# hamidthri/navbot_ppo

Measured on AMD Instinct MI355X. Metric: env_steps_per_sec, higher is better.
Workload: dtype f32; 1 GPU; BASELINE configs[1]: 4096 envs/GPU, stage_1 (32 segments), 10 beams, PPO mlp64x2, rollout=512, 50 full-batch epochs, episode cap 500; n_envs_total=4096, n_envs_per_gpu=4096, rollout_len=512, epochs=50, policy=mlp64x2, parallelism=env-shard dp1, update_arith=bf16x3, rollout=persistent kernel (navsim_rollout_mlp64)

## Files before the change

navbot_ppo_amd/csrc/ppo_mlp64_x3s.h:

```cpp
#pragma once

namespace x3s {

typedef unsigned u32x4 __attribute__((ext_vector_type(4)));
typedef unsigned u32x2 __attribute__((ext_vector_type(2)));
typedef short s16x4 __attribute__((ext_vector_type(4)));
typedef float v4f __attribute__((ext_vector_type(4)));

constexpr int SW = 4;
constexpr int kPieceB = 32 * 128;
constexpr int kImgB = 3 * kPieceB;

struct SmemS {
    uint16_t W2p[3][H][H];
    uint16_t W2Tp[3][H][H];
    uint16_t W1p[3][H][16];
    float b1[H], b2[H], w3[H], w4[H];
    unsigned char img[SW][2][kImgB];
};
static_assert(sizeof(SmemS) <= 160 * 1024, "LDS");
static_assert(offsetof(SmemS, img) % 128 == 0 && kImgB % 128 == 0, "image bases keep the low 7 address bits of a lane offset (the XOR swizzles)");
static_assert(sizeof(SmemS::img) >= 4 * ((Layout<16>::P_ACTOR + 6) & ~3) * sizeof(float), "reduction rows fit the images");
static_assert(sizeof(SmemS::img) / SW >= 96 * 64 * sizeof(float), "lane partials fit a wave's images");

#ifndef X3S_GUARD
#define X3S_GUARD ""
#endif
#define X3S_G "s_nop 0\n\t"
#define X3S_MFMA32_V_AV(acc, A, B) asm volatile(X3S_GUARD "v_mfma_f32_32x32x16_bf16 %0, %1, %2, %0" : "+v"(acc) : "a"(A), "v"(B))
#define X3S_MFMA32_V_AA(acc, A, B) asm volatile(X3S_GUARD "v_mfma_f32_32x32x16_bf16 %0, %1, %2, %0" : "+v"(acc) : "a"(A), "a"(B))
#define X3S_MFMA32G_V_AV(acc, A, B) asm volatile(X3S_G "v_mfma_f32_32x32x16_bf16 %0, %1, %2, %0" : "+v"(acc) : "a"(A), "v"(B))
#define X3S_MFMA32G_V_AA(acc, A, B) asm volatile(X3S_G "v_mfma_f32_32x32x16_bf16 %0, %1, %2, %0" : "+v"(acc) : "a"(A), "a"(B))
#define X3S_MFMA32_VZ_AV(acc, A, B) asm volatile(X3S_G "v_mfma_f32_32x32x16_bf16 %0, %1, %2, 0" : "=&v"(acc) : "a"(A), "v"(B))
#define X3S_MFMA32_VZ_AA(acc, A, B) asm volatile(X3S_G "v_mfma_f32_32x32x16_bf16 %0, %1, %2, 0" : "=&v"(acc) : "a"(A), "a"(B))
#define X3S_MFMA32_A_AV(acc, A, B) asm volatile(X3S_GUARD "v_mfma_f32_32x32x16_bf16 %0, %1, %2, %0" : "+a"(acc) : "a"(A), "v"(B))
#define X3S_MFMA32_AZ_AV(acc, A, B) asm volatile(X3S_G "v_mfma_f32_32x32x16_bf16 %0, %1, %2, 0" : "=&a"(acc) : "a"(A), "v"(B))
#define X3S_MFMA32_A_AA(acc, A, B) asm volatile(X3S_GUARD "v_mfma_f32_32x32x16_bf16 %0, %1, %2, %0" : "+a"(acc) : "a"(A), "a"(B))
#define X3S_MFMA16_A_AA(acc, A, B) asm volatile(X3S_GUARD "v_mfma_f32_16x16x32_bf16 %0, %1, %2, %0" : "+a"(acc) : "a"(A), "a"(B))
#define X3S_MFMA16_V_AA(acc, A, B) asm volatile(X3S_GUARD "v_mfma_f32_16x16x32_bf16 %0, %1, %2, %0" : "+v"(acc) : "a"(A), "a"(B))
#define X3S_MFMA16G_V_AA(acc, A, B) asm volatile(X3S_G "v_mfma_f32_16x16x32_bf16 %0, %1, %2, %0" : "+v"(acc) : "a"(A), "a"(B))
#define X3S_MFMA16_A_VA(acc, A, B) asm volatile(X3S_GUARD "v_mfma_f32_16x16x32_bf16 %0, %1, %2, %0" : "+a"(acc) : "v"(A), "a"(B))
#define X3S_MFMA16_V_VA(acc, A, B) asm volatile(X3S_GUARD "v_mfma_f32_16x16x32_bf16 %0, %1, %2, %0" : "+v"(acc) : "v"(A), "a"(B))
#define X3S_MFMA16G_A_AA(acc, A, B) asm volatile(X3S_G "v_mfma_f32_16x16x32_bf16 %0, %1, %2, %0" : "+a"(acc) : "a"(A), "a"(B))
#define X3S_MFMA16_A_AV(acc, A, B) asm volatile(X3S_GUARD "v_mfma_f32_16x16x32_bf16 %0, %1, %2, %0" : "+a"(acc) : "a"(A), "v"(B))

#define X3S_REP10(F, b) F(b + 0); F(b + 1); F(b + 2); F(b + 3); F(b + 4); F(b + 5); F(b + 6); F(b + 7); F(b + 8); F(b + 9);


__device__ __forceinline__ void split_a(unsigned& p0, float& ra, float& rb, const float a, const float b) {
    asm volatile("v_cvt_pk_bf16_f32 %0, %3, %4\n\t"
                 "v_lshlrev_b32 %1, 16, %0\n\t"
                 "v_and_b32 %2, 0xffff0000, %0\n\t"
                 "v_sub_f32 %1, %3, %1\n\t"
                 "v_sub_f32 %2, %4, %2"
                 : "=&v"(p0), "=&v"(ra), "=&v"(rb) : "v"(a), "v"(b));
}
__device__ __forceinline__ void split_b(unsigned& p1, unsigned& p2, const float ra, const float rb) {
    float t0, t1;
    asm volatile("v_cvt_pk_bf16_f32 %0, %4, %5\n\t"
                 "v_lshlrev_b32 %2, 16, %0\n\t"
                 "v_and_b32 %3, 0xffff0000, %0\n\t"
                 "v_sub_f32 %2, %4, %2\n\t"
                 "v_sub_f32 %3, %5, %3\n\t"
                 "v_cvt_pk_bf16_f32 %1, %2, %3"
                 : "=&v"(p1), "=&v"(p2), "=&v"(t0), "=&v"(t1) : "v"(ra), "v"(rb));
}
__device__ __forceinline__ void relu4(float (&h)[16], const f32x16& c, const int g) {
    float y0, y1, y2, y3;
    asm volatile("v_max_i32 %0, %4, 0\n\tv_max_i32 %1, %5, 0\n\tv_max_i32 %2, %6, 0\n\tv_max_i32 %3, %7, 0"
                 : "=&v"(y0), "=&v"(y1), "=&v"(y2), "=&v"(y3) : "v"(c[4 * g]), "v"(c[4 * g + 1]), "v"(c[4 * g + 2]), "v"(c[4 * g + 3]));
    h[4 * g] = y0; h[4 * g + 1] = y1; h[4 * g + 2] = y2; h[4 * g + 3] = y3;
}
template <bool ACTOR>
__device__ __forceinline__ void dot4(float& z3, float& z4, const float (&h)[16], const int g, const v4f w3, const v4f w4) {
    if constexpr (ACTOR)
        asm volatile("v_fmac_f32 %0, %2, %6\n\tv_fmac_f32 %1, %2, %10\n\t"
                     "v_fmac_f32 %0, %3, %7\n\tv_fmac_f32 %1, %3, %11\n\t"
                     "v_fmac_f32 %0, %4, %8\n\tv_fmac_f32 %1, %4, %12\n\t"
                     "v_fmac_f32 %0, %5, %9\n\tv_fmac_f32 %1, %5, %13"
                     : "+v"(z3), "+v"(z4)
                     : "v"(h[4 * g]), "v"(h[4 * g + 1]), "v"(h[4 * g + 2]), "v"(h[4 * g + 3]), "v"(w3.x), "v"(w3.y), "v"(w3.z), "v"(w3.w),
                       "v"(w4.x), "v"(w4.y), "v"(w4.z), "v"(w4.w));
    else
        asm volatile("v_fmac_f32 %0, %1, %5\n\tv_fmac_f32 %0, %2, %6\n\tv_fmac_f32 %0, %3, %7\n\tv_fmac_f32 %0, %4, %8"
                     : "+v"(z3)
                     : "v"(h[4 * g]), "v"(h[4 * g + 1]), "v"(h[4 * g + 2]), "v"(h[4 * g + 3]), "v"(w3.x), "v"(w3.y), "v"(w3.z), "v"(w3.w));
}
template <bool ACTOR>
__device__ __forceinline__ void dh2_value(float& h, float& pw3, float& pw4, float& pb2, const float g3, const float g4, const float w3,
                                          const float w4) {
    float d;
    if constexpr (ACTOR)
        asm volatile("v_fmac_f32 %1, %0, %5\n\t"
                     "v_fmac_f32 %2, %0, %6\n\t"
                     "v_mul_f32 %4, %6, %8\n\t"
                     "v_fmac_f32 %4, %5, %7\n\t"
                     "v_cmp_lt_f32 vcc, 0, %0\n\t"
                     "v_cndmask_b32 %0, 0, %4, vcc\n\t"
                     "v_add_f32 %3, %3, %0"
                     : "+v"(h), "+v"(pw3), "+v"(pw4), "+v"(pb2), "=&v"(d) : "v"(g3), "v"(g4), "v"(w3), "v"(w4) : "vcc");
    else
        asm volatile("v_fmac_f32 %1, %0, %4\n\t"
                     "v_mul_f32 %3, %4, %5\n\t"
                     "v_cmp_lt_f32 vcc, 0, %0\n\t"
                     "v_cndmask_b32 %0, 0, %3, vcc\n\t"
                     "v_add_f32 %2, %2, %0"
                     : "+v"(h), "+v"(pw3), "+v"(pb2), "=&v"(d) : "v"(g3), "v"(w3) : "vcc");
}

__device__ __forceinline__ void mask4(float& y0, float& y1, float& y2, float& y3, const float x0, const float x1, const float x2,
                                      const float x3, const unsigned w0, const unsigned w1) {
    asm volatile("v_cmp_ne_u16 vcc, 0, %8\n\t"
                 "v_cndmask_b32 %0, 0, %4, vcc\n\t"
                 "v_cmp_lt_u32 vcc, 0xffff, %8\n\t"
                 "v_cndmask_b32 %1, 0, %5, vcc\n\t"
                 "v_cmp_ne_u16 vcc, 0, %9\n\t"
                 "v_cndmask_b32 %2, 0, %6, vcc\n\t"
                 "v_cmp_lt_u32 vcc, 0xffff, %9\n\t"
                 "v_cndmask_b32 %3, 0, %7, vcc"
                 : "=&v"(y0), "=&v"(y1), "=&v"(y2), "=&v"(y3) : "v"(x0), "v"(x1), "v"(x2), "v"(x3), "v"(w0), "v"(w1) : "vcc");
}

struct P3 {
    u32x4 p[3];
};

__device__ __forceinline__ int fswz(const int m) { return (m & 3) | ((((m >> 2) ^ (m >> 3)) & 1) << 2) | ((((m >> 1) ^ (m >> 3)) & 1) << 3); }

typedef __attribute__((address_space(3))) s16x4* lds_s16x4;
__device__ __forceinline__ u32x2 tr_read(const unsigned char* p) {
    const s16x4 v = __builtin_amdgcn_ds_read_tr16_b64_v4i16((lds_s16x4)p);
    u32x2 r;
    __builtin_memcpy(&r, &v, 8);
    return r;
}
__device__ __forceinline__ u32x4 cat(const u32x2 lo, const u32x2 hi) { return u32x4{lo.x, lo.y, hi.x, hi.y}; }

template <bool ACTOR>
__device__ __forceinline__ void pass_body(SmemS& sm, const float* __restrict__ params, const unsigned char* __restrict__ prep,
                                          const float* __restrict__ act, const float* __restrict__ logp_old,
                                          const float* __restrict__ rtg, const float* __restrict__ adv, long long M, float var,
                                          float clip, float inv_n, float* __restrict__ partial, float* __restrict__ stats_partial) {
    using L = Layout<16>;
    constexpr int OFF_W1 = L::OFF_W1, OFF_B1 = L::OFF_B1, OFF_W2 = L::OFF_W2, OFF_B2 = L::OFF_B2, OFF_W3 = L::OFF_W3, OFF_B3 = L::OFF_B3,
                  OFF_W4 = L::OFF_W4, OFF_B4 = L::OFF_B4;
    constexpr int P = ACTOR ? L::P_ACTOR : L::P_CRITIC;
    constexpr int NT = 64 * SW, kTileBytes = XPad<16>::kTileBytes, kRowsBytes = XPad<16>::kRowsBytes;
    const int tid = threadIdx.x, lane = tid & 63, wave = __builtin_amdgcn_readfirstlane(tid >> 6);
    const int l31 = lane & 31, lhi = lane >> 5, l15 = lane & 15, kk = lane >> 4;

#ifdef X3S_EXPERIMENT_COPY_PROLOGUE
    for (int k = tid; k < (int)offsetof(SmemS, img) / 16; k += NT)
        reinterpret_cast<u32x4*>(&sm)[k] = reinterpret_cast<const u32x4*>(prep)[k + (ACTOR ? 0 : (int)offsetof(SmemS, img) / 16)];
#else
    for (int k = tid; k < H * H / 2; k += NT) {
        const int r = (2 * k) / H, c = (2 * k) % H;
        uint32_t p0, p1, p2;
        bf16x3::split_pair(params[OFF_W2 + r * H + c], params[OFF_W2 + r * H + c + 1], p0, p1, p2);
        const uint32_t pc[3] = {p0, p1, p2};
#pragma unroll
        for (int i = 0; i < 3; ++i) {
            *reinterpret_cast<uint32_t*>(&sm.W2p[i][0][0] + wslot(r, kpos(c))) = pc[i];
            (&sm.W2Tp[i][0][0])[wslot(c, kpos(r))] = (uint16_t)(pc[i] & 0xffffu);
            (&sm.W2Tp[i][0][0])[wslot(c + 1, kpos(r))] = (uint16_t)(pc[i] >> 16);
        }
    }
    for (int k = tid; k < H * 16 / 2; k += NT) {
        const int r = (2 * k) / 16, c = (2 * k) % 16;
        uint32_t p0, p1, p2;
        bf16x3::split_pair(params[OFF_W1 + r * 16 + c], params[OFF_W1 + r * 16 + c + 1], p0, p1, p2);
        *reinterpret_cast<uint32_t*>(&sm.W1p[0][r][c]) = p0;
        *reinterpret_cast<uint32_t*>(&sm.W1p[1][r][c]) = p1;
        *reinterpret_cast<uint32_t*>(&sm.W1p[2][r][c]) = p2;
    }
    if (tid < H) {
        sm.b1[tid] = params[OFF_B1 + tid];
        sm.b2[tid] = params[OFF_B2 + tid];
        sm.w3[tid] = params[OFF_W3 + tid];
        sm.w4[tid] = ACTOR ? params[OFF_W4 + tid] : 0.f;
    }
#endif
    const float b3 = params[OFF_B3];
    const float b4 = ACTOR ? params[OFF_B4] : 0.f;
    __syncthreads();

    unsigned char* const smb = reinterpret_cast<unsigned char*>(&sm);
    const int img0 = (int)offsetof(SmemS, img) + wave * 2 * kImgB;
    constexpr int IMG_H = 0, IMG_D = kImgB;
    const int st_base = img0 + l31 * 128 + ((fswz(l31) ^ lhi) << 3);
    auto st_off = [&](const int t, const int j, const int b) { return st_base ^ ((8 * t + 4 * j + 2 * b) << 3); };
    const int g_row = 8 * lhi + (l15 >> 2), g_quad = 4 * ((lane >> 4) & 1) + (lane & 3);
    const int g_base0 = img0 + g_row * 128 + ((g_quad ^ fswz(g_row)) << 3), g_base1 = img0 + (g_row + 4) * 128 + ((g_quad ^ fswz(g_row + 4)) << 3);
    auto g_off = [&](const int t, const int s, const int rd) { return ((rd ? g_base1 : g_base0) ^ (t << 6)) + s * 2048; };
    const int h_row = 8 * kk + (l15 >> 2), h_quad = lane & 3;
    const int h_base0 = img0 + h_row * 128 + ((h_quad ^ fswz(h_row)) << 3), h_base1 = img0 + (h_row + 4) * 128 + ((h_quad ^ fswz(h_row + 4)) << 3);
    auto ldw = [&](const uint16_t* base, const int tt, const int s, const int i) {
        return *reinterpret_cast<const u32x4*>(base + i * H * H + wslot(32 * tt + l31, 16 * s + 8 * lhi));
    };
    const int vec_off = 4 * lhi;
    auto ldv = [&](const float* v, const int t, const int g) { return *reinterpret_cast<const v4f*>(v + 32 * t + 8 * g + vec_off); };

    f32x16 aW2[2][2];
    v4f aW1[4], aB1[4];
#pragma unroll
    for (int a = 0; a < 2; ++a)
#pragma unroll
        for (int b = 0; b < 2; ++b) aW2[a][b] = zero16();
#pragma unroll
    for (int u = 0; u < 4; ++u) aW1[u] = aB1[u] = v4f{0.f, 0.f, 0.f, 0.f};
    float pb2[2][16], pw3[2][16], pw4[2][16];
#pragma unroll
    for (int t = 0; t < 2; ++t)
#pragma unroll
        for (int r = 0; r < 16; ++r) pb2[t][r] = pw3[t][r] = pw4[t][r] = 0.f;
    float adb3 = 0.f, adb4 = 0.f, st0 = 0.f, st1 = 0.f, st2 = 0.f, st3 = 0.f;
    auto keep_w2 = [&]() {
        asm volatile("" : "+a"(aW2[0][0]), "+a"(aW2[0][1]), "+a"(aW2[1][0]), "+a"(aW2[1][1]), "+a"(aW1[0]), "+a"(aW1[1]), "+a"(aW1[2]), "+a"(aW1[3]));
    };
    u32x4 ones = {0x3f803f80u, 0x3f803f80u, 0x3f803f80u, 0x3f803f80u};
    asm volatile("" : "+a"(ones));

    const long long n_tiles = (M + 31) / 32;
    const long long gw = (long long)blockIdx.x * SW + wave, stride = (long long)gridDim.x * SW;
    u32x4 xp[3], xbn[3];
    auto keep_cols = [&]() { asm volatile("" : "+a"(xbn[0]), "+a"(xbn[1]), "+a"(xbn[2])); };
    float pre_a0 = 0.f, pre_a1 = 0.f, pre_lp = 0.f, pre_t = 0.f;
    auto request_rows = [&](long long t) {
        asm volatile("" : "+s"(t));
        const unsigned char* r = prep + (size_t)t * kTileBytes + ((l31 * 3) * 16 + 8 * lhi) * 2;
        asm volatile("global_load_dwordx4 %0, %3, off\n\tglobal_load_dwordx4 %1, %3, off offset:32\n\tglobal_load_dwordx4 %2, %3, off offset:64"
                     : "=a"(xp[0]), "=a"(xp[1]), "=a"(xp[2]) : "v"(r));
    };
    auto request_cols = [&](const long long t) {
        const unsigned char* c = prep + (size_t)t * kTileBytes + kRowsBytes + (l15 * 32 + 8 * kk) * 2;
        asm volatile("global_load_dwordx4 %0, %3, off\n\tglobal_load_dwordx4 %1, %3, off offset:1024\n\tglobal_load_dwordx4 %2, %3, off offset:2048"
                     : "=a"(xbn[0]), "=a"(xbn[1]), "=a"(xbn[2]) : "v"(c));
    };
    auto request_scalars = [&](const long long t) {
        if constexpr (ACTOR) {
            const long long m = t * 32 + l31;
            if (m < M) {
                const float2 a = reinterpret_cast<const float2*>(act)[m];
                pre_a0 = a.x;
                pre_a1 = a.y;
                pre_lp = logp_old[m];
                pre_t = adv[m];
            }
        } else {
            int l = l31;
            long long ts = t;
            asm volatile("" : "+v"(l), "+s"(ts));
            const long long m = ts * 32 + l;
            pre_t = rtg[m < M ? m : M - 1];
        }
    };
    auto landed = [&]() {
        asm volatile("s_waitcnt vmcnt(0)" : "+a"(xp[0]), "+a"(xp[1]), "+a"(xp[2]), "+a"(xbn[0]), "+a"(xbn[1]), "+a"(xbn[2]));
    };
    static_assert(kTileBytes == 6144 && kRowsBytes == 3072, "offsets of the asm loads: pieces 32 bytes apart in a row, 1024 in the columns");

    struct G1Ops {
        P3 da[4];
    };
    auto g1_gather_pair = [&](G1Ops& o, const int q, const int hb0, const int hb1) {
        const int u = q / 3, i = q % 3;
        o.da[u].p[i] = cat(tr_read(smb + (hb0 ^ (u << 5)) + IMG_D + i * kPieceB), tr_read(smb + (hb1 ^ (u << 5)) + IMG_D + i * kPieceB));
    };
    auto g1_step = [&](const int k, const G1Ops& o, const u32x4 (&xb)[3], const bool guard = false) {
        const int t1 = k / 18, q = k % 18, u = 2 * t1 + (q & 1), e = q >> 1;
        constexpr int kind[9] = {0, 1, 0, 0, 1, 0, 0, 1, 0};
        constexpr int ai[9] = {2, 2, 1, 0, 1, 1, 0, 0, 0};
        constexpr int bi[9] = {0, 0, 1, 2, 0, 0, 1, 0, 0};
        if (guard) {
            if (kind[e]) { X3S_MFMA16G_V_AA(aB1[u], o.da[u].p[ai[e]], ones); }
            else { X3S_MFMA16G_A_AA(aW1[u], o.da[u].p[ai[e]], xb[bi[e]]); }
        } else {
            if (ACTOR) {
                if (kind[e]) { X3S_MFMA16_V_AA(aB1[u], o.da[u].p[ai[e]], ones); }
                else { X3S_MFMA16_A_AA(aW1[u], o.da[u].p[ai[e]], xb[bi[e]]); }
            } else {
                if (kind[e]) { X3S_MFMA16_V_VA(aB1[u], o.da[u].p[ai[e]], ones); }
                else { X3S_MFMA16_A_VA(aW1[u], o.da[u].p[ai[e]], xb[bi[e]]); }
            }
        }
    };
    auto store_pieces = [&](const int img, const int t, const int j, const P3& q) {
#pragma unroll
        for (int i = 0; i < 3; ++i) {
            *reinterpret_cast<u32x2*>(smb + st_off(t, j, 0) + img + i * kPieceB) = u32x2{q.p[i].x, q.p[i].y};
            *reinterpret_cast<u32x2*>(smb + st_off(t, j, 1) + img + i * kPieceB) = u32x2{q.p[i].z, q.p[i].w};
        }
    };
    struct SplitState {
        float ra[4], rb[4];
    };
    auto split_block = [&](const float (&c)[16], const int j, const int b, P3& q, SplitState& ss) {
        const int pr = b >> 1;
        if ((b & 1) == 0) {
            unsigned p0;
            split_a(p0, ss.ra[pr], ss.rb[pr], c[8 * j + 2 * pr], c[8 * j + 2 * pr + 1]);
            q.p[0][pr] = p0;
        } else {
            unsigned p1, p2;
            split_b(p1, p2, ss.ra[pr], ss.rb[pr]);
            q.p[1][pr] = p1;
            q.p[2][pr] = p2;
        }
    };

    f32x16 c1[2], c2[2];
    float h1[2][16];
    P3 hb[4];
    u32x4 wn[2][3], wa[2][3];
    SplitState ss1;
    auto g2_step = [&](const int k, const P3 (&dA)[2][2], const P3 (&hB)[2][2], f32x16 (&aW2)[2][2]) {
        const int t2 = k / 24, sk = (k / 12) & 1, e = (k % 12) >> 1, t1 = k & 1;
        constexpr int ai[6] = {2, 1, 0, 1, 0, 0}, bi[6] = {0, 1, 2, 0, 1, 0};
        X3S_MFMA32_A_AA(aW2[t2][t1], dA[t2][sk].p[ai[e]], hB[t1][sk].p[bi[e]]);
    };
    auto b1_to_c1 = [&](const int q) {
        const v4f b = ldv(sm.b1, q >> 2, q & 3);
        c1[q >> 2][4 * (q & 3)] = b.x; c1[q >> 2][4 * (q & 3) + 1] = b.y; c1[q >> 2][4 * (q & 3) + 2] = b.z; c1[q >> 2][4 * (q & 3) + 3] = b.w;
    };
    auto b2_to_c2 = [&](const int q) {
        const v4f b = ldv(sm.b2, q >> 2, q & 3);
        c2[q >> 2][4 * (q & 3)] = b.x; c2[q >> 2][4 * (q & 3) + 1] = b.y; c2[q >> 2][4 * (q & 3) + 2] = b.z; c2[q >> 2][4 * (q & 3) + 3] = b.w;
    };
    auto ld_wa = [&](const int t, const int i) { wa[t][i] = *reinterpret_cast<const u32x4*>(&sm.W1p[i][32 * t + l31][8 * lhi]); };
    auto ld_wn = [&](const int t, const int i) { wn[t][i] = ldw(&sm.W2p[0][0][0], t, 0, i); };
    auto f1_mfma = [&](const int j) {
        const int t = j / 6, e = j % 6;
        constexpr int wi[6] = {2, 1, 0, 1, 0, 0}, xi[6] = {0, 1, 2, 0, 1, 0};
        if (e == 0) { X3S_MFMA32G_V_AA(c1[t], wa[t][wi[e]], xp[xi[e]]); } else { X3S_MFMA32_V_AA(c1[t], wa[t][wi[e]], xp[xi[e]]); }
    };
    auto ahead_work = [&](const int n, const bool alone) {
        if (n == 11 || n == 13) ld_wa(0, (n - 11) / 2);
        if (n == 15 || n == 17) ld_wa(1, (n - 15) / 2);
        if (n == 19) { ld_wa(0, 2); ld_wa(1, 2); }
        if (n >= 22 && n <= 29) b1_to_c1(n - 22);
        if (n == 42) { ld_wn(0, 0); ld_wn(1, 0); ld_wn(0, 1); ld_wn(1, 1); }
        if (n == 43) {
            ld_wn(0, 2); ld_wn(1, 2);
            if (alone) asm volatile("s_nop 7" : "+v"(c1[0]));
            relu4(h1[0], c1[0], 0);
        }
        if (n == 44) relu4(h1[0], c1[0], 1);
        if (n >= 45 && n <= 52) { split_block(h1[0], 0, n - 45, hb[0], ss1); b2_to_c2(n - 45); }
        if (n == 53) relu4(h1[0], c1[0], 2);
        if (n == 54) relu4(h1[0], c1[0], 3);
        if (n >= 55 && n <= 58) relu4(h1[1], c1[1], n - 55);
    };

    for (int k = lane; k < kImgB / 16; k += 64) reinterpret_cast<u32x4*>(smb + img0 + IMG_D)[k] = u32x4{0u, 0u, 0u, 0u};
    bool have_prev = false;
    if (gw < n_tiles) {
        request_rows(gw);
        request_cols(gw);
        request_scalars(gw);
        auto slot = [&](const int n) {
            if (n == 36) landed();
            if (n >= 36 && n < 48) f1_mfma(n - 36);
            ahead_work(n, true);
        };
        X3S_REP10(slot, 10) X3S_REP10(slot, 20) X3S_REP10(slot, 30) X3S_REP10(slot, 40) X3S_REP10(slot, 50)
    }
    for (long long tile = gw; tile < n_tiles; tile += stride) {
        const bool valid = tile * 32 + l31 < M;
        const float cur_a0 = pre_a0, cur_a1 = pre_a1, cur_lp = pre_lp, cur_t = pre_t;
        const long long tile1 = tile + stride < n_tiles ? tile + stride : tile;

        G1Ops g1o;
        float h2[2][16];
        float z3 = 0.f, z4 = 0.f;
        {
            u32x4 wk[4][2];
            SplitState ss;
#pragma unroll
            for (int s = 0; s < 3; ++s) {
                u32x4 w[2][3];
#pragma unroll
                for (int i = 0; i < 3; ++i) { w[0][i] = wn[0][i]; w[1][i] = wn[1][i]; }
                keep_w2();
                keep_cols();
                auto filler = [&](const int slot) {
                    if (slot >= 1 && slot <= 8) split_block(h1[(s + 1) >> 1], (s + 1) & 1, slot - 1, hb[s + 1], ss);
                    if (slot == 0 || slot == 4 || slot == 9) {
                        const int i = slot == 0 ? 0 : slot == 4 ? 1 : 2;
                        wn[0][i] = ldw(&sm.W2p[0][0][0], 0, s + 1, i);
                        wn[1][i] = ldw(&sm.W2p[0][0][0], 1, s + 1, i);
                    }
                    if (slot == 9) store_pieces(IMG_H, s >> 1, s & 1, hb[s]);
                };
                if (s == 0) { X3S_MFMA32G_V_AV(c2[0], w[0][2], hb[s].p[0]); } else { X3S_MFMA32_V_AV(c2[0], w[0][2], hb[s].p[0]); }
                filler(0);
                if (s == 0) { X3S_MFMA32G_V_AV(c2[1], w[1][2], hb[s].p[0]); } else { X3S_MFMA32_V_AV(c2[1], w[1][2], hb[s].p[0]); }
                filler(1);
                X3S_MFMA32_V_AV(c2[0], w[0][1], hb[s].p[1]); filler(2);
                X3S_MFMA32_V_AV(c2[1], w[1][1], hb[s].p[1]); filler(3);
                X3S_MFMA32_V_AV(c2[0], w[0][0], hb[s].p[2]); filler(4);
                X3S_MFMA32_V_AV(c2[1], w[1][0], hb[s].p[2]); filler(5);
                X3S_MFMA32_V_AV(c2[0], w[0][1], hb[s].p[0]); filler(6);
                X3S_MFMA32_V_AV(c2[1], w[1][1], hb[s].p[0]); filler(7);
                X3S_MFMA32_V_AV(c2[0], w[0][0], hb[s].p[1]); filler(8);
                X3S_MFMA32_V_AV(c2[1], w[1][0], hb[s].p[1]); filler(9);
            }
            int hb0 = h_base0, hb1 = h_base1;
            asm volatile("" : "+v"(hb0), "+v"(hb1));
            int gq = 0;
            auto gather = [&]() { g1_gather_pair(g1o, gq, hb0, hb1); ++gq; };
            auto ld_wk = [&](const int s, const int t) { wk[s][t] = ldw(&sm.W2p[0][0][0], t, s, 0); };
            keep_w2();
            keep_cols();
            X3S_MFMA32_V_AV(c2[0], wn[0][2], hb[3].p[0]); ld_wk(0, 0); ld_wk(1, 0);
            X3S_MFMA32_V_AV(c2[0], wn[0][1], hb[3].p[1]); ld_wk(2, 0); ld_wk(3, 0);
            X3S_MFMA32_V_AV(c2[0], wn[0][0], hb[3].p[2]); gather(); gather();
            X3S_MFMA32_V_AV(c2[0], wn[0][1], hb[3].p[0]); gather(); gather();
            X3S_MFMA32_V_AV(c2[0], wn[0][0], hb[3].p[1]); gather(); gather();
            X3S_MFMA32_V_AV(c2[0], wk[0][0], hb[0].p[0]); gather(); gather();
            X3S_MFMA32_V_AV(c2[0], wk[1][0], hb[1].p[0]); gather(); gather();
            X3S_MFMA32_V_AV(c2[0], wk[2][0], hb[2].p[0]); gather();
            X3S_MFMA32_V_AV(c2[0], wk[3][0], hb[3].p[0]); gather();
            v4f hw3[4], hw4[4] = {};
            auto ld_hw = [&](const int g) {
                hw3[g] = ldv(sm.w3, 0, g);
                if (ACTOR) hw4[g] = ldv(sm.w4, 0, g);
            };
            X3S_MFMA32_V_AV(c2[1], wn[1][2], hb[3].p[0]); ld_wk(0, 1); ld_wk(1, 1); ld_hw(0);
            X3S_MFMA32_V_AV(c2[1], wn[1][1], hb[3].p[1]); ld_wk(2, 1); ld_wk(3, 1); ld_hw(1);
            X3S_MFMA32_V_AV(c2[1], wn[1][0], hb[3].p[2]); store_pieces(IMG_H, 1, 1, hb[3]);
            X3S_MFMA32_V_AV(c2[1], wn[1][1], hb[3].p[0]); relu4(h2[0], c2[0], 0); relu4(h2[0], c2[0], 1);
            X3S_MFMA32_V_AV(c2[1], wn[1][0], hb[3].p[1]); relu4(h2[0], c2[0], 2); relu4(h2[0], c2[0], 3);
#pragma unroll
            for (int s = 0; s < 4; ++s) {
                X3S_MFMA32_V_AV(c2[1], wk[s][1], hb[s].p[0]);
                dot4<ACTOR>(z3, z4, h2[0], s, hw3[s], hw4[s]);
                if (s < 2) ld_hw(s + 2);
            }
        }

        int g1k = 0;
        keep_w2();
        {
            v4f hw3[4], hw4[4] = {};
            g1_step(g1k++, g1o, xbn);
            hw3[0] = ldv(sm.w3, 1, 0); hw3[1] = ldv(sm.w3, 1, 1);
            if (ACTOR) { hw4[0] = ldv(sm.w4, 1, 0); hw4[1] = ldv(sm.w4, 1, 1); }
            g1_step(g1k++, g1o, xbn);
            hw3[2] = ldv(sm.w3, 1, 2); hw3[3] = ldv(sm.w3, 1, 3);
            if (ACTOR) { hw4[2] = ldv(sm.w4, 1, 2); hw4[3] = ldv(sm.w4, 1, 3); }
            g1_step(g1k++, g1o, xbn);
            relu4(h2[1], c2[1], 0); relu4(h2[1], c2[1], 1);
            g1_step(g1k++, g1o, xbn);
            relu4(h2[1], c2[1], 2); relu4(h2[1], c2[1], 3);
#pragma unroll
            for (int g = 0; g < 4; ++g) {
                g1_step(g1k++, g1o, xbn);
                dot4<ACTOR>(z3, z4, h2[1], g, hw3[g], hw4[g]);
            }
        }
        float g3 = 0.f, g4 = 0.f;
        {
            z3 += __shfl_xor(z3, 32, 64);
            if (ACTOR) z4 += __shfl_xor(z4, 32, 64);
            const float own = (lhi == 0) ? 1.f : 0.f;
            if (valid) {
                z3 += b3;
                z4 += b4;
#ifdef MLP64_DEBUG_Z
                if (lhi == 0) {
                    float* const dbg = partial + (size_t)200 * P;
                    dbg[tile * 32 + l31] = z3;
                    if (ACTOR) dbg[M + tile * 32 + l31] = z4;
                }
#endif
                if (ACTOR) {
                    const float mu0 = 1.0f / (1.0f + expf(-z3));
                    const float mu1 = tanhf(z4);
                    const float d0 = cur_a0 - mu0, d1 = cur_a1 - mu1;
                    const float lp = -0.5f * ((d0 * d0 + d1 * d1) / var) - 1.8378770664093453f - logf(var);
                    const float lr = lp - cur_lp;
                    const float ratio = expf(lr);
                    const float A = cur_t;
                    const float s1 = ratio * A;
                    const float rc = fminf(fmaxf(ratio, 1.0f - clip), 1.0f + clip);
                    const float s2 = rc * A;
                    st0 += own * -fminf(s1, s2);
                    st2 += own * ((ratio - 1.0f) - lr);
                    st3 += (fabsf(ratio - 1.0f) > clip) ? own : 0.f;
                    const bool inside = (ratio >= 1.0f - clip) && (ratio <= 1.0f + clip);
                    const float dL_dratio = (inside || s1 < s2) ? -A : 0.f;
                    const float dL_dlp = dL_dratio * ratio * inv_n;
                    g3 = dL_dlp * (d0 / var) * (mu0 * (1.0f - mu0));
                    g4 = dL_dlp * (d1 / var) * (1.0f - mu1 * mu1);
                } else {
                    const float e = z3 - cur_t;
                    st1 += own * (e * e);
                    g3 = 2.0f * e * inv_n;
                }
            }
            adb3 += own * g3;
            adb4 += own * g4;
#ifdef MLP64_DEBUG_Z
            if (valid && lhi == 0) {
                float* const dbg = partial + (size_t)200 * P;
                dbg[2 * M + tile * 32 + l31] = g3;
                if (ACTOR) dbg[3 * M + tile * 32 + l31] = g4;
            }
#endif
        }
        {
            v4f wn3 = ldv(sm.w3, 0, 0), wn4 = ACTOR ? ldv(sm.w4, 0, 0) : v4f{0.f, 0.f, 0.f, 0.f};
#pragma unroll
            for (int q = 0; q < 8; ++q) {
                const int t = q >> 2, g = q & 3;
                const v4f w = wn3, v = wn4;
                if (q < 7) {
                    wn3 = ldv(sm.w3, (q + 1) >> 2, (q + 1) & 3);
                    if (ACTOR) wn4 = ldv(sm.w4, (q + 1) >> 2, (q + 1) & 3);
                }
                const float wv3[4] = {w.x, w.y, w.z, w.w}, wv4[4] = {v.x, v.y, v.z, v.w};
#pragma unroll
                for (int j = 0; j < 4; ++j) {
                    const int r = 4 * g + j;
                    dh2_value<ACTOR>(h2[t][r], pw3[t][r], pw4[t][r], pb2[t][r], g3, g4, wv3[j], wv4[j]);
                    if (g1k < 36 && (j & 1)) g1_step(g1k++, g1o, xbn);
                }
                if (g1k < 36 && (g & 1)) g1_step(g1k++, g1o, xbn);
            }
        }

        f32x16 c3[2];
        P3 hB[2][2], dA[2][2];
        u32x2 mw[8];
        float d1[2][16];
        auto d_mask = [&](const int k) {
            const int t = k >> 2, r0 = 8 * ((k >> 1) & 1) + 4 * (k & 1);
            mask4(d1[t][r0], d1[t][r0 + 1], d1[t][r0 + 2], d1[t][r0 + 3], c3[t][r0], c3[t][r0 + 1], c3[t][r0 + 2], c3[t][r0 + 3], mw[k].x, mw[k].y);
        };
        {
            P3 db[4];
            u32x4 wk[4][2], wt[2][3];
            SplitState ss;
#pragma unroll
            for (int i = 0; i < 3; ++i) {
                wt[0][i] = ldw(&sm.W2Tp[0][0][0], 0, 0, i);
                wt[1][i] = ldw(&sm.W2Tp[0][0][0], 1, 0, i);
            }
#pragma unroll
            for (int b = 0; b < 8; ++b) {
                g1_step(g1k++, g1o, xbn);
                split_block(h2[0], 0, b, db[0], ss);
            }
#pragma unroll
            for (int s = 0; s < 4; ++s) {
                u32x4 w[2][3];
#pragma unroll
                for (int i = 0; i < 3; ++i) { w[0][i] = wt[0][i]; w[1][i] = wt[1][i]; }
                keep_w2();
                auto filler = [&](const int slot) {
                    if (s == 0 && slot == 0) request_cols(tile);
                    if (s == 0 && slot == 1) request_rows(tile1);
                    if (s == 3 && slot == 0) request_scalars(tile1);
                    if (s < 3 && slot >= 1 && slot <= 8) split_block(h2[(s + 1) >> 1], (s + 1) & 1, slot - 1, db[s + 1], ss);
                    if (s == 3 && slot < 8) wk[slot >> 1][slot & 1] = ldw(&sm.W2Tp[0][0][0], slot & 1, slot >> 1, 0);
                    if (slot == 2 || slot == 5 || slot == 8) {
                        const int q = 3 * s + (slot - 2) / 3, t = q / 6, sk = (q / 3) & 1, i = q % 3;
                        hB[t][sk].p[i] = cat(tr_read(smb + g_off(t, sk, 0) + IMG_H + i * kPieceB), tr_read(smb + g_off(t, sk, 1) + IMG_H + i * kPieceB));
                    }
                    if (s == 3 && (slot == 3 || slot == 4 || slot == 6 || slot == 7)) {
                        const int k0 = 2 * (slot - 3 - (slot > 4));
#pragma unroll
                        for (int k = k0; k < k0 + 2; ++k)
                            mw[k] = *reinterpret_cast<const u32x2*>(smb + st_off(k >> 2, (k >> 1) & 1, k & 1) + IMG_H);
                    }
                    if (s < 3 && (slot == 0 || slot == 4 || slot == 9)) {
                        const int i = slot == 0 ? 0 : slot == 4 ? 1 : 2;
                        wt[0][i] = ldw(&sm.W2Tp[0][0][0], 0, s + 1, i);
                        wt[1][i] = ldw(&sm.W2Tp[0][0][0], 1, s + 1, i);
                    }
                    if (slot == 9) store_pieces(IMG_D, s >> 1, s & 1, db[s]);
                };
                if (s == 0) { X3S_MFMA32_VZ_AV(c3[0], w[0][2], db[s].p[0]); } else { X3S_MFMA32_V_AV(c3[0], w[0][2], db[s].p[0]); }
                filler(0);
                if (s == 0) { X3S_MFMA32_VZ_AV(c3[1], w[1][2], db[s].p[0]); } else { X3S_MFMA32_V_AV(c3[1], w[1][2], db[s].p[0]); }
                filler(1);
                X3S_MFMA32_V_AV(c3[0], w[0][1], db[s].p[1]); filler(2);
                X3S_MFMA32_V_AV(c3[1], w[1][1], db[s].p[1]); filler(3);
                X3S_MFMA32_V_AV(c3[0], w[0][0], db[s].p[2]); filler(4);
                X3S_MFMA32_V_AV(c3[1], w[1][0], db[s].p[2]); filler(5);
                X3S_MFMA32_V_AV(c3[0], w[0][1], db[s].p[0]); filler(6);
                X3S_MFMA32_V_AV(c3[1], w[1][1], db[s].p[0]); filler(7);
                X3S_MFMA32_V_AV(c3[0], w[0][0], db[s].p[1]); filler(8);
                X3S_MFMA32_V_AV(c3[1], w[1][0], db[s].p[1]); filler(9);
            }
            int dq = 0;
            auto gather_d = [&]() {
                const int t = dq / 6, sk = (dq / 3) & 1, i = dq % 3;
                dA[t][sk].p[i] = cat(tr_read(smb + g_off(t, sk, 0) + IMG_D + i * kPieceB), tr_read(smb + g_off(t, sk, 1) + IMG_D + i * kPieceB));
                ++dq;
            };
#pragma unroll
            for (int s = 0; s < 4; ++s) {
                X3S_MFMA32_V_AV(c3[0], wk[s][0], db[s].p[0]);
                gather_d(); gather_d();
            }
#pragma unroll
            for (int s = 0; s < 4; ++s) {
                X3S_MFMA32_V_AV(c3[1], wk[s][1], db[s].p[0]);
                if (s < 2) { gather_d(); gather_d(); }
                else d_mask(s - 2);
            }
        }

        {
            P3 eb[4];
            SplitState ss;
            auto d_work = [&](const int n) {
                if (n == 0 || n == 1) d_mask(2 + n);
                if (n == 20 || n == 21) d_mask(4 + n - 20);
                if (n == 31 || n == 32) d_mask(6 + n - 31);
                const int s = n < 11 ? 0 : n < 20 ? 1 : n < 31 ? 2 : 3, n0 = s == 0 ? 2 : s == 1 ? 11 : s == 2 ? 22 : 33;
                if (n >= n0 && n < n0 + 8) split_block(d1[s >> 1], s & 1, n - n0, eb[s], ss);
                if (n == n0 + 8) store_pieces(IMG_D, s >> 1, s & 1, eb[s]);
            };
            auto slot = [&](const int n) {
                if (n == 36) landed();
                if (n < 36) g2_step(n, dA, hB, aW2);
                else if (n < 48) f1_mfma(n - 36);
                else g2_step(n - 12, dA, hB, aW2);
                d_work(n);
                ahead_work(n, false);
            };
            X3S_REP10(slot, 0) X3S_REP10(slot, 10) X3S_REP10(slot, 20) X3S_REP10(slot, 30) X3S_REP10(slot, 40) X3S_REP10(slot, 50)
        }
        have_prev = true;
    }
    if (have_prev) {
        G1Ops g1o;
#pragma unroll
        for (int q = 0; q < 12; ++q) g1_gather_pair(g1o, q, h_base0, h_base1);
#pragma unroll
        for (int k = 0; k < 36; ++k) g1_step(k, g1o, xbn, true);
    }

    __syncthreads();
    float rb2[2], rw3[2], rw4[2];
    {
        float* const scr = reinterpret_cast<float*>(&sm.img[wave][0][0]);
#pragma unroll
        for (int t = 0; t < 2; ++t)
#pragma unroll
            for (int r = 0; r < 16; ++r) {
                scr[(0 * 32 + 16 * t + r) * 64 + lane] = pb2[t][r];
                scr[(1 * 32 + 16 * t + r) * 64 + lane] = pw3[t][r];
                scr[(2 * 32 + 16 * t + r) * 64 + lane] = pw4[t][r];
            }
        __builtin_amdgcn_fence(__ATOMIC_RELEASE, "wavefront");
        __builtin_amdgcn_wave_barrier();
        const int row = l31, hi = (row >> 2) & 1, r = (row & 3) + 4 * (row >> 3), t = lhi;
        float s[3] = {0.f, 0.f, 0.f};
#pragma unroll
        for (int v = 0; v < 3; ++v) {
            const float* src = scr + (v * 32 + 16 * t + r) * 64 + 32 * hi;
#pragma unroll
            for (int m = 0; m < 32; m += 4) {
                const v4f q = *reinterpret_cast<const v4f*>(src + m);
                s[v] += (q.x + q.y) + (q.z + q.w);
            }
        }
        rb2[0] = s[0]; rw3[0] = s[1]; rw4[0] = s[2];
        rb2[1] = rw3[1] = rw4[1] = 0.f;
    }
    __syncthreads();

    constexpr int RP = (P + 3 + 3) & ~3;
    float s3 = adb3, s4 = adb4, sA = ACTOR ? st0 : st1, sB = st2, sC = st3;
#pragma unroll
    for (int o = 32; o >= 1; o >>= 1) {
        s3 += __shfl_xor(s3, o, 64); s4 += __shfl_xor(s4, o, 64);
        sA += __shfl_xor(sA, o, 64); sB += __shfl_xor(sB, o, 64); sC += __shfl_xor(sC, o, 64);
    }
    float* const red0 = reinterpret_cast<float*>(&sm.img[0][0][0]);
    float* const rowp = red0 + wave * RP;
    {
        auto put = [&](int idx, float v) { rowp[idx] = v; };
#pragma unroll
        for (int t2 = 0; t2 < 2; ++t2)
#pragma unroll
            for (int t1 = 0; t1 < 2; ++t1)
#pragma unroll
                for (int r = 0; r < 16; ++r) put(OFF_W2 + (32 * t2 + c_row(r, lane)) * H + 32 * t1 + l31, aW2[t2][t1][r]);
        put(OFF_B2 + 32 * lhi + l31, rb2[0]);
        put(OFF_W3 + 32 * lhi + l31, rw3[0]);
        if (ACTOR) put(OFF_W4 + 32 * lhi + l31, rw4[0]);
#pragma unroll
        for (int u = 0; u < 4; ++u) {
#pragma unroll
            for (int r = 0; r < 4; ++r) put(OFF_W1 + (16 * u + 4 * kk + r) * 16 + l15, aW1[u][r]);
            if (l15 == 0) {
#pragma unroll
                for (int r = 0; r < 4; ++r) put(OFF_B1 + 16 * u + 4 * kk + r, aB1[u][r]);
            }
        }
        if (lane == 0) {
            put(OFF_B3, s3);
            if (ACTOR) put(OFF_B4, s4);
            put(P + 0, sA);
            put(P + 1, sB);
            put(P + 2, sC);
        }
    }
    __syncthreads();
    float* out = partial + (size_t)blockIdx.x * P;
    const float* red = red0;
    for (int k = tid; k < P; k += NT) out[k] = (red[k] + red[RP + k]) + (red[2 * RP + k] + red[3 * RP + k]);
    if (tid < 3) stats_partial[blockIdx.x * 4 + tid] = (red[P + tid] + red[RP + P + tid]) + (red[2 * RP + P + tid] + red[3 * RP + P + tid]);
}

}

__global__ __launch_bounds__(64 * x3s::SW) void NAVPPO_KL_KERNEL(mlp64_pass_both_x3s)(const float* __restrict__ params, const unsigned char* __restrict__ prep,
                                                                    const float* __restrict__ act, const float* __restrict__ logp_old,
                                                                    const float* __restrict__ rtg, const float* __restrict__ adv,
                                                                    long long M, float var, float clip, float inv_n, int net_mask,
                                                                    float* __restrict__ partial_a, float* __restrict__ stats_partial_a,
                                                                    float* __restrict__ partial_c, float* __restrict__ stats_partial_c NAVPPO_KL_PARAM) {
    __shared__ __attribute__((aligned(128))) x3s::SmemS sm;
    NAVPPO_KL_GATE();
    if (net_mask & 1) x3s::pass_body<true>(sm, params, prep, act, logp_old, rtg, adv, M, var, clip, inv_n, partial_a, stats_partial_a);
    if (net_mask == 3) __syncthreads();
    if (net_mask & 2) x3s::pass_body<false>(sm, params + Layout<16>::P_ACTOR, prep, act, logp_old, rtg, adv, M, var, clip, inv_n, partial_c, stats_partial_c);
}
```

Baseline: 55.82 million env-steps/s.

## Interleave actor/critic pass order across paired blocks in fused PPO update kernel

Blocks whose index has the X3S_PAIR bit set now run the critic pass first and then the actor pass, using a remapped block index so each network's partial output slots stay unique. The goal is to spread the two networks' different instruction mixes and memory streams across concurrently resident blocks instead of having every block run actor then critic in lockstep. It also zero-initialises the accumulators from an opaque register value, moves the final g1 drain inside the have_prev scope with an s_nop fence, and hides threadIdx from the compiler to control register allocation. The two passes are now selected inside a runtime phase loop, which can raise code size and register pressure.

```diff
diff --git a/navbot_ppo_amd/csrc/ppo_mlp64_x3s.h b/navbot_ppo_amd/csrc/ppo_mlp64_x3s.h
--- a/navbot_ppo_amd/csrc/ppo_mlp64_x3s.h
+++ b/navbot_ppo_amd/csrc/ppo_mlp64_x3s.h
@@ -140,13 +140,16 @@
 __device__ __forceinline__ void pass_body(SmemS& sm, const float* __restrict__ params, const unsigned char* __restrict__ prep,
                                           const float* __restrict__ act, const float* __restrict__ logp_old,
                                           const float* __restrict__ rtg, const float* __restrict__ adv, long long M, float var,
-                                          float clip, float inv_n, float* __restrict__ partial, float* __restrict__ stats_partial) {
+                                          float clip, float inv_n, float* __restrict__ partial, float* __restrict__ stats_partial,
+                                          const int block) {
     using L = Layout<16>;
     constexpr int OFF_W1 = L::OFF_W1, OFF_B1 = L::OFF_B1, OFF_W2 = L::OFF_W2, OFF_B2 = L::OFF_B2, OFF_W3 = L::OFF_W3, OFF_B3 = L::OFF_B3,
                   OFF_W4 = L::OFF_W4, OFF_B4 = L::OFF_B4;
     constexpr int P = ACTOR ? L::P_ACTOR : L::P_CRITIC;
     constexpr int NT = 64 * SW, kTileBytes = XPad<16>::kTileBytes, kRowsBytes = XPad<16>::kRowsBytes;
-    const int tid = threadIdx.x, lane = tid & 63, wave = __builtin_amdgcn_readfirstlane(tid >> 6);
+    int tid = threadIdx.x;
+    asm volatile("" : "+v"(tid));
+    const int lane = tid & 63, wave = __builtin_amdgcn_readfirstlane(tid >> 6);
     const int l31 = lane & 31, lhi = lane >> 5, l15 = lane & 15, kk = lane >> 4;
 
 #ifdef X3S_EXPERIMENT_COPY_PROLOGUE
@@ -200,20 +203,24 @@
     const int vec_off = 4 * lhi;
     auto ldv = [&](const float* v, const int t, const int g) { return *reinterpret_cast<const v4f*>(v + 32 * t + 8 * g + vec_off); };
 
+    float zf = 0.f;
+    asm volatile("" : "+v"(zf));
     f32x16 aW2[2][2];
     v4f aW1[4], aB1[4];
 #pragma unroll
     for (int a = 0; a < 2; ++a)
 #pragma unroll
-        for (int b = 0; b < 2; ++b) aW2[a][b] = zero16();
-#pragma unroll
-    for (int u = 0; u < 4; ++u) aW1[u] = aB1[u] = v4f{0.f, 0.f, 0.f, 0.f};
+        for (int b = 0; b < 2; ++b)
+#pragma unroll
+            for (int r = 0; r < 16; ++r) aW2[a][b][r] = zf;
+#pragma unroll
+    for (int u = 0; u < 4; ++u) aW1[u] = aB1[u] = v4f{zf, zf, zf, zf};
     float pb2[2][16], pw3[2][16], pw4[2][16];
 #pragma unroll
     for (int t = 0; t < 2; ++t)
 #pragma unroll
-        for (int r = 0; r < 16; ++r) pb2[t][r] = pw3[t][r] = pw4[t][r] = 0.f;
-    float adb3 = 0.f, adb4 = 0.f, st0 = 0.f, st1 = 0.f, st2 = 0.f, st3 = 0.f;
+        for (int r = 0; r < 16; ++r) pb2[t][r] = pw3[t][r] = pw4[t][r] = zf;
+    float adb3 = zf, adb4 = zf, st0 = zf, st1 = zf, st2 = zf, st3 = zf;
     auto keep_w2 = [&]() {
         asm volatile("" : "+a"(aW2[0][0]), "+a"(aW2[0][1]), "+a"(aW2[1][0]), "+a"(aW2[1][1]), "+a"(aW1[0]), "+a"(aW1[1]), "+a"(aW1[2]), "+a"(aW1[3]));
     };
@@ -221,7 +228,7 @@
     asm volatile("" : "+a"(ones));
 
     const long long n_tiles = (M + 31) / 32;
-    const long long gw = (long long)blockIdx.x * SW + wave, stride = (long long)gridDim.x * SW;
+    const long long gw = (long long)block * SW + wave, stride = (long long)gridDim.x * SW;
     u32x4 xp[3], xbn[3];
     auto keep_cols = [&]() { asm volatile("" : "+a"(xbn[0]), "+a"(xbn[1]), "+a"(xbn[2])); };
     float pre_a0 = 0.f, pre_a1 = 0.f, pre_lp = 0.f, pre_t = 0.f;
@@ -363,7 +370,6 @@
             ahead_work(n, true);
         };
         X3S_REP10(slot, 10) X3S_REP10(slot, 20) X3S_REP10(slot, 30) X3S_REP10(slot, 40) X3S_REP10(slot, 50)
-    }
     for (long long tile = gw; tile < n_tiles; tile += stride) {
         const bool valid = tile * 32 + l31 < M;
         const float cur_a0 = pre_a0, cur_a1 = pre_a1, cur_lp = pre_lp, cur_t = pre_t;
@@ -641,6 +647,8 @@
         for (int q = 0; q < 12; ++q) g1_gather_pair(g1o, q, h_base0, h_base1);
 #pragma unroll
         for (int k = 0; k < 36; ++k) g1_step(k, g1o, xbn, true);
+        asm volatile("s_nop 7" : "+a"(aW1[0]), "+a"(aW1[1]), "+a"(aW1[2]), "+a"(aW1[3]), "+v"(aB1[0]), "+v"(aB1[1]), "+v"(aB1[2]), "+v"(aB1[3]));
+    }
     }
 
     __syncthreads();
@@ -711,13 +719,18 @@
         }
     }
     __syncthreads();
-    float* out = partial + (size_t)blockIdx.x * P;
+    float* out = partial + (size_t)block * P;
     const float* red = red0;
     for (int k = tid; k < P; k += NT) out[k] = (red[k] + red[RP + k]) + (red[2 * RP + k] + red[3 * RP + k]);
-    if (tid < 3) stats_partial[blockIdx.x * 4 + tid] = (red[P + tid] + red[RP + P + tid]) + (red[2 * RP + P + tid] + red[3 * RP + P + tid]);
-}
-
-}
+    if (tid < 3) stats_partial[block * 4 + tid] = (red[P + tid] + red[RP + P + tid]) + (red[2 * RP + P + tid] + red[3 * RP + P + tid]);
+}
+
+}
+
+#ifndef X3S_PAIR
+#define X3S_PAIR 8
+#endif
+static_assert(X3S_PAIR >= 0 && (X3S_PAIR & (X3S_PAIR - 1)) == 0, "X3S_PAIR is 0 or one bit of the block index");
 
 __global__ __launch_bounds__(64 * x3s::SW) void NAVPPO_KL_KERNEL(mlp64_pass_both_x3s)(const float* __restrict__ params, const unsigned char* __restrict__ prep,
                                                                     const float* __restrict__ act, const float* __restrict__ logp_old,
@@ -727,7 +740,27 @@
                                                                     float* __restrict__ partial_c, float* __restrict__ stats_partial_c NAVPPO_KL_PARAM) {
     __shared__ __attribute__((aligned(128))) x3s::SmemS sm;
     NAVPPO_KL_GATE();
-    if (net_mask & 1) x3s::pass_body<true>(sm, params, prep, act, logp_old, rtg, adv, M, var, clip, inv_n, partial_a, stats_partial_a);
+#if X3S_PAIR
+    const int b = blockIdx.x;
+    const bool paired = net_mask == 3 && gridDim.x % (2 * X3S_PAIR) == 0;
+    const bool critic_first = paired && (b & X3S_PAIR);
+#pragma nounroll
+    for (int phase = 0; phase < 2; ++phase) {
+        int blk = b;
+        asm volatile("" : "+s"(blk));
+        if (__builtin_expect((phase == 0) != critic_first, 1)) {
+            if (net_mask & 1) x3s::pass_body<true>(sm, params, prep, act, logp_old, rtg, adv, M, var, clip, inv_n, partial_a, stats_partial_a, blk);
+        } else {
+            if (net_mask & 2)
+                x3s::pass_body<false>(sm, params + Layout<16>::P_ACTOR, prep, act, logp_old, rtg, adv, M, var, clip, inv_n, partial_c, stats_partial_c,
+                                      paired ? blk ^ X3S_PAIR : blk);
+        }
+        if (phase == 0 && net_mask == 3) __syncthreads();
+    }
+#else
+    if (net_mask & 1) x3s::pass_body<true>(sm, params, prep, act, logp_old, rtg, adv, M, var, clip, inv_n, partial_a, stats_partial_a, blockIdx.x);
     if (net_mask == 3) __syncthreads();
-    if (net_mask & 2) x3s::pass_body<false>(sm, params + Layout<16>::P_ACTOR, prep, act, logp_old, rtg, adv, M, var, clip, inv_n, partial_c, stats_partial_c);
-}
+    if (net_mask & 2)
+        x3s::pass_body<false>(sm, params + Layout<16>::P_ACTOR, prep, act, logp_old, rtg, adv, M, var, clip, inv_n, partial_c, stats_partial_c, blockIdx.x);
+#endif
+}
```

Measured after the change: 57.14 million env-steps/s (median of 6 runs). 1.02x the previous value.
